# rdesc/autorally

Hardware: AMD Instinct MI355X
Metric: trajectory rollouts/s per MPPI solve (higher is better)
Workload: dtype f32

## Files before the change

autorally_amd/csrc/group_roles.hpp:

```cpp
#pragma once

#include "mppi_device.hpp"
#include "noise_device.hpp"

namespace mppi {

constexpr int kGRing = 16;
constexpr int kGCtlChunk = 4;

template <class SH>
struct GroupRoles {
  static constexpr int kPose = SH::NW, kCost = SH::NW + 1, kCtl = SH::NW + 2, kRng = SH::NW + 3;
  static constexpr int kWaves = SH::NW + 4;
  static_assert(kWaves <= (int)(sizeof(SH::fin) / sizeof(int)), "fin[]");
  static_assert(SH::kR == 16 || SH::kR == 8, "rollouts per group");
};
template <class SH>
__device__ __forceinline__ int group_j(int slot) { return slot & (SH::kR - 1); }
template <class SH>
__device__ __forceinline__ bool group_real(int slot) { return slot < SH::kR; }

template <class SH>
__device__ __forceinline__ int group_seq_min(SH &sh)
{
// ... 194 lines not shown
      y = fmaf(sd1, a.dt, y);
      yaw = fmaf(sd2, a.dt, yaw);
    }
    if (t > 0) {
      while (cdone < t - kGRing && --budget > 0) cdone = lds_peek(a_cd);
      if (lane < kRolloutsPerWave) *reinterpret_cast<float2 *>(&sh.tex[(t - 1) & (kGRing - 1)][lane][0]) = make_float2(tf_p, tb_p);
      lds_publish(a_mypub, t);
    }
    tf_p = tf; tb_p = tb;
  }
  spin_finish(budget, lds_addr(&sh.fail[0]), lds_addr(&sh.fin[R::kPose]));
}

template <int Q>
__device__ __forceinline__ float quad_bc(float v)
{
  return __int_as_float(__builtin_amdgcn_mov_dpp(__float_as_int(v), Q * 0x55, 0xF, 0xF, false));
}
__device__ __forceinline__ void quad_chain(float v, float d, float dt, int q, float &vq, float &v_out)
{
  const float v1 = fmaf(quad_bc<0>(d), dt, v);
  const float v2 = fmaf(quad_bc<1>(d), dt, v1);
  const float v3 = fmaf(quad_bc<2>(d), dt, v2);
  v_out = fmaf(quad_bc<3>(d), dt, v3);
  const float lo = (q == 0) ? v : v1, hi = (q == 2) ? v2 : v3;
  vq = (q < 2) ? lo : hi;
}
template <class SH, bool AFFINE>
__device__ __forceinline__ void group_pose_wave4(const RolloutArgs &a, SH &sh, const float x0, const float y0, const float yaw0,
                                                 const int budget_cut = 0);
template <class SH, bool AFFINE>
__device__ __forceinline__ void group_pose_wave4(const RolloutArgs &a, SH &sh)
{
  group_pose_wave4<SH, AFFINE>(a, sh, a.state[0], a.state[1], a.state[2]);
}
template <class SH, bool AFFINE>
__device__ __forceinline__ void group_pose_wave4(const RolloutArgs &a, SH &sh, const float x0, const float y0, const float yaw0,
                                                 const int budget_cut)
{
  using R = GroupRoles<SH>;
  constexpr int NSW = SH::NSW;
  static_assert(kRolloutsPerWave == 16 && kGRing >= 8, "lane = 4 j + q");
  const int lane = threadIdx.x & 63;
  const int j = group_j<SH>(lane >> 2), q = lane & 3;
  const int T = a.T;
  const uint32_t a_seq0 = lds_addr(&sh.xseq[0][0]);
  const uint32_t a_cd = lds_addr(&sh.cost_done[0]);
  const uint32_t a_mypub = lds_addr(&sh.pose_pub[lane]);
  float x = x0, y = y0, yaw = yaw0;
  int budget = spin_budget_init(a.spin_budget, T, a.fault_wave == R::kPose + 1 || budget_cut != 0), seen = 0, cdone = 0;
  for (int t0 = 0; t0 < T; t0 += 4) {
    const int t = t0 + q;
    const int tend = min(t0 + 4, T);
    const int need = (tend - 1) * NSW + 1;
    while (seen < need && --budget > 0) {
      seen = SH::kRecByAll ? group_seq_min(sh) : lds_peek(a_seq0);
      if (seen < need) __builtin_amdgcn_s_sleep(1);
    }
    const float4 r0 = *reinterpret_cast<const float4 *>(&sh.rec[t & (kGRing - 1)][j][0]);
    float yaw_q, yaw_n, x_q, x_n, y_q, y_n;
    quad_chain(yaw, a.negate_yaw_der ? -r0.w : r0.w, a.dt, q, yaw_q, yaw_n);
    float spsi, cpsi, tf = 0.0f, tb = 0.0f;
#ifdef MPPI_DIAG_NOPOSE
    spsi = 0.0f; cpsi = 1.0f;
#else
    sincos_fast(yaw_q, spsi, cpsi);
#endif
    quad_chain(x, fmaf(cpsi, r0.y, -(spsi * r0.z)), a.dt, q, x_q, x_n);
    quad_chain(y, fmaf(spsi, r0.y, cpsi * r0.z), a.dt, q, y_q, y_n);
#ifdef MPPI_DIAG_NOPOSE
    tf = x_q; tb = y_q;
#else
    const float st[3] = {x_q, y_q, yaw_q};
    track_fetch<AFFINE>(a.cost, st, cpsi, spsi, tf, tb);
#endif
    x = x_n; y = y_n; yaw = yaw_n;
    while (cdone < tend - kGRing && --budget > 0) cdone = lds_peek(a_cd);
    if (t < T) *reinterpret_cast<float2 *>(&sh.tex[t & (kGRing - 1)][j][0]) = make_float2(tf, tb);
    lds_publish(a_mypub, tend);
  }
  spin_finish(budget, lds_addr(&sh.fail[0]), lds_addr(&sh.fin[R::kPose]));
}

template <class SH>
__device__ __forceinline__ float group_settle(SH &sh, int budget, float J)
{
  using R = GroupRoles<SH>;
  const int lane = threadIdx.x & 63;
  const uint32_t a_fin = lds_addr(&sh.fin[(lane < R::kWaves) ? lane : 0]);
  for (;;) {
    const int v = (lane == R::kCost) ? 1 : lds_peek_lanes(a_fin);
    const bool all = __builtin_amdgcn_ballot_w64(v != 0) == ~0ull;
    if (all || --budget <= 0) break;
    __builtin_amdgcn_s_sleep(1);
  }
  if (budget <= 0 || lds_peek(lds_addr(&sh.fail[0])) != 0) J = __builtin_nanf("");
  return J;
}

template <class SH, bool CTRL>
__device__ __forceinline__ void group_cost_wave(const RolloutArgs &a, SH &sh)
{
  using R = GroupRoles<SH>;
  const int lane = threadIdx.x & 63;
  static_assert(SH::kR == 16, "one step per iteration: 16-rollout groups only");
  const int j = lane & 15;
  const int k = (int)blockIdx.x * kRolloutsPerWave + j;
// ... 2 lines not shown
  const uint32_t a_pose = lds_addr(&sh.pose_pub[0]);
  int crash = 0, budget = spin_budget_init(a.spin_budget, T, a.fault_wave == R::kCost + 1), seen = 0;
  float J = 0.0f;
  for (int t = 0; t < T; t++) {
    const double rt = a.inv_t[t];
    while (seen < t + 1 && --budget > 0) {
      seen = lds_peek(a_pose);
      if (seen < t + 1) __builtin_amdgcn_s_sleep(1);
    }
    const float4 r0 = *reinterpret_cast<const float4 *>(&sh.rec[t & (kGRing - 1)][j][0]);
    const float4 r1 = *reinterpret_cast<const float4 *>(&sh.ctl_rec[t & (kGRing - 1)][j][0]);
    const float2 tx = *reinterpret_cast<const float2 *>(&sh.tex[t & (kGRing - 1)][j][0]);
    lds_publish(a_mydone, t + 1);
    const int rc = (int)((t > 0) & (fabsf(r0.x) >= kRollCrash));
#ifdef MPPI_DIAG_NOCOST
    crash |= rc;
    int crash_new = crash;
    const float Jn = J + r0.y + r1.x + tx.x + (float)rt;
#else
    CostTerms ct;
    cost_terms_a<CTRL>(a.cost, a.nu, r0.y, r0.z, r1.x, r1.y, r1.z, r1.w, ct);
    crash |= rc;
    int crash_new = crash;
    const float c = cost_terms_b(a.cost, ct, tx.x, tx.y, crash_new);
    const float Jn = running_mean(J, c, t, rt);
#endif
    J = (t > 0) ? Jn : J;
    crash = (t > 0) ? crash_new : crash;
  }
  J = group_settle(sh, budget, J);
  a.costs[k] = J + 0.0f;
}

template <int Q>
__device__ __forceinline__ int quad_bc_i(int v)
{
  return __builtin_amdgcn_mov_dpp(v, Q * 0x55, 0xF, 0xF, false);
}
template <class SH, bool CTRL>
__device__ __forceinline__ void group_cost_wave4(const RolloutArgs &a, SH &sh)
{
  using R = GroupRoles<SH>;
  const int lane = threadIdx.x & 63;
  const int j = group_j<SH>(lane >> 2), q = lane & 3;
  const int k = (int)blockIdx.x * SH::kR + j;
  const int T = a.T;
  const uint32_t a_mydone = lds_addr(&sh.cost_done[lane]);
  const uint32_t a_pose = lds_addr(&sh.pose_pub[0]);
  int crash = 0, budget = spin_budget_init(a.spin_budget, T, a.fault_wave == R::kCost + 1), seen = 0;
  float J = 0.0f;
  for (int t0 = 0; t0 < T; t0 += 4) {
    const int t = t0 + q;
    const int tend = min(t0 + 4, T);
    while (seen < tend && --budget > 0) {
      seen = lds_peek(a_pose);
      if (seen < tend) __builtin_amdgcn_s_sleep(1);
    }
    const float4 r0 = *reinterpret_cast<const float4 *>(&sh.rec[t & (kGRing - 1)][j][0]);
    const float4 r1 = *reinterpret_cast<const float4 *>(&sh.ctl_rec[t & (kGRing - 1)][j][0]);
    const float2 tx = *reinterpret_cast<const float2 *>(&sh.tex[t & (kGRing - 1)][j][0]);
    lds_publish(a_mydone, tend);
    const bool counted = (t > 0) & (t < T);
    int e = (int)(fabsf(r0.x) >= kRollCrash) | (int)(tx.x >= a.cost.boundary_threshold) | (int)(tx.y >= a.cost.boundary_threshold);
    e = counted ? e : 0;
    const int c0 = crash | quad_bc_i<0>(e), c1 = c0 | quad_bc_i<1>(e), c2 = c1 | quad_bc_i<2>(e), c3 = c2 | quad_bc_i<3>(e);
    const int lo = (q == 0) ? c0 : c1, hi = (q == 2) ? c2 : c3;
    int crash_q = (q < 2) ? lo : hi;
    crash = c3;
#ifdef MPPI_DIAG_NOCOST
    const float c = r0.y + r1.x + tx.x + (float)crash_q;
#else
    CostTerms ct;
    cost_terms_a<CTRL>(a.cost, a.nu, r0.y, r0.z, r1.x, r1.y, r1.z, r1.w, ct);
    const float c = cost_terms_b(a.cost, ct, tx.x, tx.y, crash_q);
#endif
#pragma unroll
    for (int l = 0; l < 4; l++) {
      const int tl = t0 + l;
      const float cl = (l == 0) ? quad_bc<0>(c) : (l == 1) ? quad_bc<1>(c) : (l == 2) ? quad_bc<2>(c) : quad_bc<3>(c);
      if (tl > 0 && tl < T) {
#ifdef MPPI_DIAG_NOCOST
        J = J + cl + (float)a.inv_t[tl];
#else
        J = running_mean(J, cl, tl, a.inv_t[tl]);
#endif
      }
    }
  }
  J = group_settle(sh, budget, J);
  if (q == 0 && group_real<SH>(lane >> 2)) a.costs[k] = J + 0.0f;
}

}
```

autorally_amd/csrc/rollout_lds128.hip:

```cpp
#include "group_roles.hpp"
#include "m44_core.hpp"
#include "mppi_kernels.hpp"

namespace mppi {

struct Lds128Net {
  int n_layers;
  int layers[8];
};

struct Lds128Shared {
  static constexpr int NW = 4;
  static constexpr int NSW = 1;
  static constexpr int kR = 16;
  static constexpr bool kRecByAll = true;
  int xseq[NW][64];
  float rec[kGRing][kRolloutsPerWave][4];
  int cost_done[64];
  float ctl_b1[kGRing][64];
  float ctl_rec[kGRing][kRolloutsPerWave][4];
  int ctl_pub[64];
  float tex[kGRing][kRolloutsPerWave][2];
  int pose_pub[64];
  float eps[kGRing][kRolloutsPerWave][2];
  int rng_pub[64];
  int fail[4];
  int fin[8];
  float gstate[8];
  int gate_open[8];
  float dump[NW][64 * kGRing];
};
constexpr size_t kLds128ImageOffset = (sizeof(Lds128Shared) + 15) & ~(size_t)15;
constexpr size_t kLds128MaxBytes = 160 * 1024;

__host__ __device__ inline int lds128_quads_of(int nin) { return (nin + 3) >> 2; }
__host__ __device__ inline int lds128_halves_of(int nout) { return nout > 64 ? 2 : 1; }

__device__ __forceinline__ void lds128_pin_reads() { asm volatile("" ::: "memory"); }

template <int Q>
__device__ __forceinline__ void lds128_chain1(m44_f4 &d, const float (&T0)[4], const float (&T1)[4], m44_f4 (&w)[kLds44Ahead],
                                              const m44_f4 *p, const int nq)
{
  if constexpr (Q < 32) {
    if (Q > 0 && Q >= nq) return;
    const m44_f4 x = w[Q % kLds44Ahead];
    if constexpr (Q + kLds44Ahead < 32) w[Q % kLds44Ahead] = p[(Q + kLds44Ahead) * 64];
    lds128_pin_reads();
    const float (&T)[4] = Q < 16 ? T0 : T1;
    d = __builtin_amdgcn_mfma_f32_4x4x1f32(T[0], x[0], d, 4, Q & 15, 0);
    d = __builtin_amdgcn_mfma_f32_4x4x1f32(T[1], x[1], d, 4, Q & 15, 0);
    d = __builtin_amdgcn_mfma_f32_4x4x1f32(T[2], x[2], d, 4, Q & 15, 0);
    d = __builtin_amdgcn_mfma_f32_4x4x1f32(T[3], x[3], d, 4, Q & 15, 0);
    lds128_chain1<Q + 1>(d, T0, T1, w, p, nq);
  }
}

template <int Q>
__device__ __forceinline__ void lds128_chain2(m44_f4 &d0, m44_f4 &d1, const float (&T0)[4], const float (&T1)[4],
                                              m44_f4 (&w)[kLds44Ahead], const m44_f4 *p, const int nq)
{
  if constexpr (Q < 32) {
    if (Q > 0 && Q >= nq) return;
    constexpr int S = 2 * Q;
    const m44_f4 x0 = w[S % kLds44Ahead];
    if constexpr (S + kLds44Ahead < 64) w[S % kLds44Ahead] = p[(S + kLds44Ahead) * 64];
    const m44_f4 x1 = w[(S + 1) % kLds44Ahead];
    if constexpr (S + 1 + kLds44Ahead < 64) w[(S + 1) % kLds44Ahead] = p[(S + 1 + kLds44Ahead) * 64];
// ... 324 lines not shown
```

autorally_amd/csrc/rollout_lds44.hip:

```cpp
#include "group_roles.hpp"
#include "m44_core.hpp"
#include "mppi_kernels.hpp"

namespace mppi {

struct Lds44Net {
  int n_layers;
  int layers[8];
};

struct Lds44Shared {
  static constexpr int NW = 4;
  static constexpr int NSW = 1;
  static constexpr int kR = 16;
  static constexpr bool kRecByAll = true;
  int xseq[NW][64];
  float rec[kGRing][kRolloutsPerWave][4];
  int cost_done[64];
  float ctl_b1[kGRing][64];
  float ctl_rec[kGRing][kRolloutsPerWave][4];
  int ctl_pub[64];
  float tex[kGRing][kRolloutsPerWave][2];
  int pose_pub[64];
  float eps[kGRing][kRolloutsPerWave][2];
  int rng_pub[64];
  int fail[4];
  int fin[8];
  float gstate[8];
  int gate_open[8];
  float dump[NW][64 * kGRing];
};
constexpr size_t kLds44ImageOffset = (sizeof(Lds44Shared) + 15) & ~(size_t)15;

__host__ __device__ inline int lds44_quads_of(int nin) { return (nin + 3) >> 2; }

template <int Q>
__device__ __forceinline__ void lds44_chain(m44_f4 &d, const float (&T)[4], m44_f4 (&w)[kLds44Ahead], const m44_f4 *p, const int nq)
{
  if constexpr (Q < 16) {
    if (Q > 0 && Q >= nq) return;
    const m44_f4 x = w[Q % kLds44Ahead];
    if constexpr (Q + kLds44Ahead < 16) w[Q % kLds44Ahead] = p[(Q + kLds44Ahead) * 64];
    d = __builtin_amdgcn_mfma_f32_4x4x1f32(T[0], x[0], d, 4, Q, 0);
    d = __builtin_amdgcn_mfma_f32_4x4x1f32(T[1], x[1], d, 4, Q, 0);
    d = __builtin_amdgcn_mfma_f32_4x4x1f32(T[2], x[2], d, 4, Q, 0);
    d = __builtin_amdgcn_mfma_f32_4x4x1f32(T[3], x[3], d, 4, Q, 0);
    lds44_chain<Q + 1>(d, T, w, p, nq);
  }
}

template <bool GATED>
__device__ __forceinline__ void lds44_dynamics(const RolloutArgs &a, const Lds44Net &net, Lds44Shared &sh, const m44_f4 *img, const int w)
{
  const int lane = threadIdx.x & 63;
  const int i = lane & 3, row = lane >> 4;
  const int jr = 4 * w + i;
  const bool hi = (lane & 2) != 0, od = (lane & 1) != 0;
  const int T = a.T;
  const int n_w = net.n_layers - 1;
  const m44_f4 *pk = img + lane;
  const float *pb = reinterpret_cast<const float *>(pk);
  const m44_f4 w0a = pk[kLds44BiasQuads * 64], w0b = pk[(kLds44BiasQuads + 1) * 64];
  const float bs0 = pb[0];
  const float bo = pb[((n_w - 1) >> 2) * 256 + ((n_w - 1) & 3)];
  const m44_f4 *const p1 = pk + (kLds44BiasQuads + 2) * 64;
  unsigned long long nq_all = 0;
#pragma unroll
  for (int l = 1; l < 8; l++) nq_all |= (unsigned long long)lds44_quads_of(net.layers[l]) << (5 * l);
// ... 250 lines not shown
```

autorally_amd/csrc/rollout_m44.hip:

```cpp
#include "group_roles.hpp"
#include "m44_core.hpp"
#include "mppi_kernels.hpp"

namespace mppi {

constexpr int kM44H = 64;

struct M44Shared {
  static constexpr int NW = 4;
  static constexpr int NSW = 1;
  static constexpr int kR = 16;
  static constexpr bool kRecByAll = true;
  int xseq[NW][64];
  float rec[kGRing][kRolloutsPerWave][4];
  int cost_done[64];
  float ctl_b1[kGRing][64];
  float ctl_rec[kGRing][kRolloutsPerWave][4];
  int ctl_pub[64];
  float tex[kGRing][kRolloutsPerWave][2];
  int pose_pub[64];
  float eps[kGRing][kRolloutsPerWave][2];
  int rng_pub[64];
  int fail[4];
  int fin[8];
  float gstate[8];
  int gate_open[8];
  m44_f4 wo[4][64];
  float dump[NW][64 * kGRing];
};

template <int NHID>
constexpr int m44_q_bias() { return 2; }
template <int NHID>
constexpr int m44_q_hidden() { return 2 + (NHID + 3) / 4; }
template <int NHID>
constexpr int m44_q_out() { return m44_q_hidden<NHID>() + (NHID - 1) * 16; }
template <int NHID>
constexpr int m44_q_total() { return m44_q_out<NHID>() + 5; }

template <int K>
__device__ __forceinline__ void m44_step(m44_f4 &d, const float (&T)[4], const float *w)
{
  d = __builtin_amdgcn_mfma_f32_4x4x1f32(T[K & 3], w[K], d, 4, K >> 2, 0);
}
template <int K0>
__device__ __forceinline__ void m44_steps16(m44_f4 &d, const float (&T)[4], const float *w)
{
#define S4(K) m44_step<K>(d, T, w); m44_step<K + 1>(d, T, w); m44_step<K + 2>(d, T, w); m44_step<K + 3>(d, T, w);
  S4(K0) S4(K0 + 4) S4(K0 + 8) S4(K0 + 12)
#undef S4
}
template <int CTRL>
__device__ __forceinline__ float m44_dpp_add(float acc, float src)
{
  return acc + __int_as_float(__builtin_amdgcn_update_dpp(0, __float_as_int(src), CTRL, 0xF, 0xF, true));
}
__device__ __forceinline__ float m44_out_tree(const f32x2 (&q)[4], const f32x2 (&p)[4], const float (&T)[4])
{
  f32x2 Q = q[0] * f32x2{T[0], T[0]}, P = p[0] * f32x2{T[0], T[0]};
#pragma unroll
  for (int s = 1; s < 4; s++) {
    Q = __builtin_elementwise_fma(q[s], f32x2{T[s], T[s]}, Q);
    P = __builtin_elementwise_fma(p[s], f32x2{T[s], T[s]}, P);
  }
  {
// ... 300 lines not shown
```

autorally_amd/csrc/rollout_oct.hip:

```cpp
#include "mfma_net.hpp"
#include "group_roles.hpp"
#include "mppi_kernels.hpp"

namespace mppi {

template <int H, int NHID>
struct OctShared {
  static constexpr int NW = 4;
  static constexpr int NSW = NHID;
  static constexpr int kR = 16;
  static constexpr bool kRecByAll = false;
  float xb[2][NW][64][4];
  int xseq[NW][64];
  float rec[kGRing][kRolloutsPerWave][4];
  int cost_done[64];
  float ctl_b1[kGRing][64];
  float ctl_rec[kGRing][kRolloutsPerWave][4];
  int ctl_pub[64];
  float tex[kGRing][kRolloutsPerWave][2];
  int pose_pub[64];
  float eps[kGRing][kRolloutsPerWave][2];
  int rng_pub[64];
  int fail[4];
  int fin[8];
};

__device__ __forceinline__ void oct_poll(const uint32_t (&a_seq)[3], const uint32_t (&a_x)[3], int &f, f32x4 (&oth)[3])
{
  int f0, f1, f2;
  asm volatile(
      "ds_read_b32 %0, %6\n\tds_read_b128 %3, %9\n\t"
      "ds_read_b32 %1, %7\n\tds_read_b128 %4, %10\n\t"
      "ds_read_b32 %2, %8\n\tds_read_b128 %5, %11\n\t"
      "s_waitcnt lgkmcnt(0)"
      : "=&v"(f0), "=&v"(f1), "=&v"(f2), "=&v"(oth[0]), "=&v"(oth[1]), "=&v"(oth[2])
      : "v"(a_seq[0]), "v"(a_seq[1]), "v"(a_seq[2]), "v"(a_x[0]), "v"(a_x[1]), "v"(a_x[2])
      : "memory");
  f = __builtin_amdgcn_readfirstlane(min(min(f0, f1), f2));
}

template <int H, int NHID, int W>
__device__ __forceinline__ void oct_dynamics(const RolloutArgs &a, OctShared<H, NHID> &sh)
{
  using N = MfmaNet<H, NHID>;
  constexpr int MT = N::MT, KSH = N::KSH, NSW = NHID;
  static_assert(MT == 4, "one M tile per dynamics wave: 64-wide hidden layers");
  const int lane = threadIdx.x & 63;
  const int j = lane & 15, g = lane >> 4;
  const int T = a.T;

  float A0[2], B0[4], AH[(NHID - 1) * KSH + 1], Bh[(NHID - 1) * 4 + 1], AL[KSH], BL[4];
  A0[0] = a.wpack[(W * 2 + 0) * 64 + lane];
  A0[1] = a.wpack[(W * 2 + 1) * 64 + lane];
#pragma unroll
  for (int r = 0; r < 4; r++) B0[r] = a.wpack[(N::nA + W * 4 + r) * 64 + lane] * kTanhScale;
#pragma unroll
  for (int l = 1; l < NHID; l++) {
#pragma unroll
    for (int s = 0; s < KSH; s++)
      AH[(l - 1) * KSH + s] = a.wpack[(N::nA0 + (l - 1) * N::nAH + W * KSH + s) * 64 + lane];
#pragma unroll
    for (int r = 0; r < 4; r++) Bh[(l - 1) * 4 + r] = a.wpack[(N::nA + l * MT * 4 + W * 4 + r) * 64 + lane] * kTanhScale;
  }
#pragma unroll
// ... 170 lines not shown
```

autorally_amd/csrc/rollout_row.hip:

```cpp
#include "group_roles.hpp"
#include "mppi_kernels.hpp"

namespace mppi {

#ifdef MPPI_ROW_STAMPS
__device__ unsigned long long g_row_stamps[16];
#define RSTAMP(i)                                                                                         \
  do {                                                                                                    \
    if (blockIdx.x == 0 && (threadIdx.x & 63) == 0) {                                                     \
      unsigned long long t__;                                                                             \
      asm volatile("s_memtime %0\n\ts_waitcnt lgkmcnt(0)" : "=s"(t__)::"memory");                           \
      g_row_stamps[i] = t__;                                                                              \
    }                                                                                                     \
  } while (0)
#else
#define RSTAMP(i) do { } while (0)
#endif

template <int H>
struct RowShared {
  static constexpr int NW = 4;
  static constexpr int NSW = 1;
  static constexpr bool kRecByAll = true;
  static constexpr int kR = 16;
  int xseq[NW][64];
  float rec[kGRing][kRolloutsPerWave][4];
  int cost_done[64];
  float ctl_b1[kGRing][64];
  float ctl_rec[kGRing][kRolloutsPerWave][4];
  int ctl_pub[64];
  float tex[kGRing][kRolloutsPerWave][2];
  int pose_pub[64];
  float eps[kGRing][kRolloutsPerWave][2];
  int rng_pub[64];
  int fail[4];
  int fin[8];
  float gstate[8];
  int gate_open[8];
  float dump[NW][64 * 2 + (kGRing - 1) * kRolloutsPerWave * 4];
};

template <int H, bool TREE>
struct RowWeights {
  f32x2 w1[kNetIn], w2[H], w3[TREE ? 4 : H];
  f32x2 b1s, b2s, b3;
};

constexpr int kRowPackEntries = 40;
template <int H, bool TREE>
__device__ __forceinline__ void row_load(const float *rowpack, int p, RowWeights<H, TREE> &W)
{
  static_assert(H == 32, "entry layout of pack_row_weights");
  const float4 *pk = reinterpret_cast<const float4 *>(rowpack) + p;
#pragma unroll
  for (int i = 0; i < 3; i++) {
    const float4 v = pk[i * 16];
    W.w1[2 * i] = f32x2{v.x, v.y};
    W.w1[2 * i + 1] = f32x2{v.z, v.w};
  }
#pragma unroll
  for (int i = 0; i < H / 2; i++) {
    const float4 v = pk[(3 + i) * 16];
    W.w2[2 * i] = f32x2{v.x, v.y};
    W.w2[2 * i + 1] = f32x2{v.z, v.w};
    if constexpr (!TREE) {
      const float4 u = pk[(3 + H / 2 + i) * 16];
      W.w3[2 * i] = f32x2{u.x, u.y};
      W.w3[2 * i + 1] = f32x2{u.z, u.w};
    }
  }
  const float4 b = pk[35 * 16];
  W.b1s = f32x2{b.x, b.y};
  W.b2s = f32x2{b.z, b.w};
  if constexpr (TREE) {
    const float4 u = pk[37 * 16], v = pk[38 * 16], c = pk[39 * 16];
    W.w3[0] = f32x2{u.x, u.y};
// ... 7 lines not shown
  }
}

template <int Q>
__device__ __forceinline__ float row_bc(float a)
{
  return __int_as_float(__builtin_amdgcn_mov_dpp(__float_as_int(a), 0x150 + Q, 0xF, 0xF, false));
}
template <int Q>
__device__ __forceinline__ f32x2 row_bc2(f32x2 a)
{
  return __builtin_bit_cast(f32x2, (long long)__builtin_amdgcn_mov_dpp(__builtin_bit_cast(long long, a), 0x150 + Q, 0xF, 0xF, false));
}
template <int Q>
__device__ __forceinline__ void row_dot_step(f32x2 &z, f32x2 &b, const f32x2 *w, f32x2 a)
{
  z = __builtin_elementwise_fma(w[2 * Q], f32x2{b.x, b.x}, z);
  __builtin_amdgcn_sched_barrier(0);
  const f32x2 bn = row_bc2<(Q + 1 < 16 ? Q + 1 : 15)>(a);
  __builtin_amdgcn_sched_barrier(0);
  z = __builtin_elementwise_fma(w[2 * Q + 1], f32x2{b.y, b.y}, z);
  __builtin_amdgcn_sched_barrier(0);
  b = bn;
}
__device__ __forceinline__ f32x2 row_dot_bc(const f32x2 *w, f32x2 a)
{
  f32x2 z = {0.0f, 0.0f};
  f32x2 b = row_bc2<0>(a);
  __builtin_amdgcn_sched_barrier(0);
#define RD4(Q) row_dot_step<Q>(z, b, w, a); row_dot_step<Q + 1>(z, b, w, a); row_dot_step<Q + 2>(z, b, w, a); row_dot_step<Q + 3>(z, b, w, a);
  RD4(0) RD4(4) RD4(8) RD4(12)
#undef RD4
  return z;
}

template <int CTRL>
__device__ __forceinline__ float dpp_add(float acc, float src)
{
  return acc + __int_as_float(__builtin_amdgcn_update_dpp(0, __float_as_int(src), CTRL, 0xF, 0xF, true));
}
__device__ __forceinline__ float row_out_tree(const f32x2 *w3, f32x2 a)
{
  const f32x2 ax = {a.x, a.x}, ay = {a.y, a.y};
  const f32x2 v01 = __builtin_elementwise_fma(w3[1], ay, w3[0] * ax);
  const f32x2 v23 = __builtin_elementwise_fma(w3[3], ay, w3[2] * ax);
  float v0 = dpp_add<0x128>(v01.x, v23.x);
  const float v1 = dpp_add<0x128>(v01.y, v23.y);
  v0 = dpp_add<0x141>(v0, v1);
  v0 = dpp_add<0xB1>(v0, v0);
  v0 = dpp_add<0x4E>(v0, v0);
  return v0;
}

template <int H, bool TREE, int Q>
__device__ __forceinline__ void row_step(const RolloutArgs &a, const RowWeights<H, TREE> &W, f32x2 &sp, f32x2 &un, const int t0,
                                         const uint32_t a_rec, const uint32_t a_myseq, const volatile int __attribute__((address_space(3))) *p_pub,
                                         const volatile f32x2 __attribute__((address_space(3))) *&pu,
                                         const volatile f32x2 __attribute__((address_space(3))) *p_u0, int &cp, int &budget)
{
  constexpr int kSlotF2 = kRolloutsPerWave * 2;
  constexpr uint32_t kRecStride = sizeof(float) * kRolloutsPerWave * 4;
  const int t = t0 + Q;
  const f32x2 u = un;
  const f32x2 slo = TREE ? f32x2{row_bc<0>(sp.x), row_bc<4>(sp.x)} : f32x2{row_bc<0>(sp.x), row_bc<0>(sp.y)};
  const f32x2 shi = TREE ? f32x2{row_bc<8>(sp.x), row_bc<12>(sp.x)} : f32x2{row_bc<1>(sp.x), row_bc<1>(sp.y)};
  if constexpr (TREE) asm volatile("ds_write_b32 %0, %1 offset:%2" ::"v"(a_rec), "v"(sp.x), "n"(Q * kRecStride) : "memory");
  else asm volatile("ds_write_b64 %0, %1 offset:%2" ::"v"(a_rec), "v"(sp), "n"(Q * kRecStride) : "memory");
  if constexpr (Q == 3) lds_publish(a_myseq, t + 1);
  f32x2 z = {0.0f, 0.0f};
  z = __builtin_elementwise_fma(W.w1[0], f32x2{slo.x, slo.x}, z);
  z = __builtin_elementwise_fma(W.w1[1], f32x2{slo.y, slo.y}, z);
  z = __builtin_elementwise_fma(W.w1[2], f32x2{shi.x, shi.x}, z);
  z = __builtin_elementwise_fma(W.w1[3], f32x2{shi.y, shi.y}, z);
  z = __builtin_elementwise_fma(W.w1[4], f32x2{u.x, u.x}, z);
  z = __builtin_elementwise_fma(W.w1[5], f32x2{u.y, u.y}, z);
  int cp_v = 0;
  if constexpr (Q == 0) cp_v = *p_pub;
  if constexpr (Q == 3) pu = p_u0 + ((t + 1) & (kGRing - 1)) * kSlotF2;
  constexpr int kUn = (Q == 3) ? 0 : (Q + 1) * kSlotF2;
  un = pu[kUn];
  const f32x2 a0 = tanh_bias2(z, W.b1s);
  const f32x2 a1 = tanh_bias2(row_dot_bc(W.w2, a0), W.b2s);
  const int want = t + 2;
  if constexpr (Q == 0) cp = __builtin_amdgcn_readfirstlane(cp_v);
  asm volatile("" : "+v"(un));
  if constexpr (TREE) {
    const float d = row_out_tree(W.w3, a1) + W.b3.x;
    sp.x = fmaf(d, a.dt, sp.x);
    asm volatile("" : "+v"(sp.x));
  } else {
    const f32x2 d = row_dot_bc(W.w3, a1) + W.b3;
    sp = __builtin_elementwise_fma(d, f32x2{a.dt, a.dt}, sp);
    asm volatile("" : "+v"(sp));
  }
  if (__builtin_expect(cp < want, 0)) {
    while (cp < want && --budget > 0) {
      cp = __builtin_amdgcn_readfirstlane(*p_pub);
      un = pu[kUn];
    }
    asm volatile("" : "+v"(un));
  }
}

template <int H, bool TREE, bool GATED = false>
__device__ __forceinline__ void row_dynamics(const RolloutArgs &a, RowShared<H> &sh, const int w)
{
  static_assert(H == 32, "row_dot_bc: 32 activations, two per lane of a 16-lane row");
  static_assert(kGRing % 4 == 0, "aligned chunks of four steps inside the ring");
  const int lane = threadIdx.x & 63;
  const int r = lane >> 4, p = lane & 15;
  const int jr = 4 * w + r;
  const bool odd = (p & 1) != 0;
  const int T = a.T;
  RowWeights<H, TREE> W;
  row_load<H, TREE>(a.wpack, p, W);
#pragma unroll
  for (int k = 0; k < H; k++) asm volatile("" : "+v"(W.w2[k]));
#pragma unroll
  for (int k = 0; k < (TREE ? 4 : H); k++) asm volatile("" : "+v"(W.w3[k]));

  const uint32_t a_myseq = lds_addr(&sh.xseq[w][lane]);
  typedef const volatile int __attribute__((address_space(3))) *lds_int_p;
  typedef const volatile f32x2 __attribute__((address_space(3))) *lds_f2_p;
  const lds_int_p p_pub = (lds_int_p)&sh.ctl_pub[0];
  uint32_t a_u0 = lds_addr(&sh.ctl_rec[0][jr][0]);
  asm volatile("" : "+v"(a_u0));
  const lds_f2_p p_u = (lds_f2_p)a_u0;
  const uint32_t a_rec0 = TREE ? (((p & 3) == 0) ? lds_addr(&sh.rec[0][jr][p >> 2]) : lds_addr(&sh.dump[w][2 * lane]))
                               : ((p < 2) ? lds_addr(&sh.rec[0][jr][2 * p]) : lds_addr(&sh.dump[w][2 * lane]));
  constexpr uint32_t kRecStride = sizeof(float) * kRolloutsPerWave * 4;

  int budget = spin_budget_init(a.spin_budget, T, a.fault_wave == w + 1);
  f32x2 sp;
  if constexpr (GATED) {
    const uint32_t a_go = lds_addr(&sh.gate_open[0]);
    while (lds_peek(a_go) == 0 && --budget > 0) __builtin_amdgcn_s_sleep(1);
    const volatile float *gs = sh.gstate;
    sp = TREE ? f32x2{gs[3 + (p >> 2)], 0.0f} : odd ? f32x2{gs[5], gs[6]} : f32x2{gs[3], gs[4]};
  } else {
    sp = TREE ? f32x2{a.state[3 + (p >> 2)], 0.0f} : odd ? f32x2{a.state[5], a.state[6]} : f32x2{a.state[3], a.state[4]};
  }
  if (w == 0) RSTAMP(2);
  int cp = 0;
  while ((cp = __builtin_amdgcn_readfirstlane(*p_pub)) < 1 && --budget > 0) __builtin_amdgcn_s_sleep(1);
  if (w == 0) RSTAMP(3);
  lds_f2_p pu = p_u;
  f32x2 un = pu[0];
  asm volatile("" : "+v"(un));

  const int NS = T - 1;
  for (int t0 = 0; t0 < NS; t0 += 4) {
    const uint32_t a_rec = a_rec0 + (uint32_t)(t0 & (kGRing - 1)) * kRecStride;
    row_step<H, TREE, 0>(a, W, sp, un, t0, a_rec, a_myseq, p_pub, pu, p_u, cp, budget);
    if (t0 + 1 >= NS) break;
    row_step<H, TREE, 1>(a, W, sp, un, t0, a_rec, a_myseq, p_pub, pu, p_u, cp, budget);
    if (t0 + 2 >= NS) break;
    row_step<H, TREE, 2>(a, W, sp, un, t0, a_rec, a_myseq, p_pub, pu, p_u, cp, budget);
    if (t0 + 3 >= NS) break;
    row_step<H, TREE, 3>(a, W, sp, un, t0, a_rec, a_myseq, p_pub, pu, p_u, cp, budget);
  }
  if (w == 0) RSTAMP(4);
  {
    const int t = T - 1;
    if constexpr (TREE) asm volatile("ds_write_b32 %0, %1" ::"v"(a_rec0 + (uint32_t)(t & (kGRing - 1)) * kRecStride), "v"(sp.x) : "memory");
    else asm volatile("ds_write_b64 %0, %1" ::"v"(a_rec0 + (uint32_t)(t & (kGRing - 1)) * kRecStride), "v"(sp) : "memory");
    lds_publish(a_myseq, t + 1);
  }
  spin_finish(budget, lds_addr(&sh.fail[0]), lds_addr(&sh.fin[w]));
}

template <int H, bool AFFINE, bool CTRL, bool TREE, bool GATED = false>
__device__ __forceinline__ void row_group(const RolloutArgs &a, RowShared<H> &sh)
{
  using SH = RowShared<H>;
  using R = GroupRoles<SH>;
  const int lane = threadIdx.x & 63;
  const int role = __builtin_amdgcn_readfirstlane(threadIdx.x >> 6);
  if (role == 0) RSTAMP(0);
  MrgHalf g0{0, 0, 0};
  if (role == R::kRng) g0 = group_rng_load<SH>(a);
  if (role == 0) {
#pragma unroll
    for (int w = 0; w < 4; w++) sh.xseq[w][lane] = 0;
    sh.cost_done[lane] = 0;
    sh.ctl_pub[lane] = 0;
    sh.pose_pub[lane] = 0;
    sh.rng_pub[lane] = 0;
    sh.fail[lane & 3] = 0;
    sh.fin[lane & 7] = 0;
    sh.gate_open[lane & 7] = 0;
  }
  __syncthreads();
  if (role == 0) RSTAMP(1);
#ifdef MPPI_ROW_RIDER_PRIO
  if (role >= 4) __builtin_amdgcn_s_setprio(MPPI_ROW_RIDER_PRIO);
#endif
  if (role < 4) row_dynamics<H, TREE, GATED>(a, sh, role);
  else if (role == R::kCost) { group_cost_wave4<SH, CTRL>(a, sh); RSTAMP(5); }
  else if (role == R::kCtl) { group_control_wave(a, sh, GATED ? lds_addr(&sh.gate_open[0]) : 0u); RSTAMP(6); }
  else if (role == R::kPose) {
    if constexpr (GATED) {
      const int shut = group_gate_wait(a, sh);
      const volatile float *gs = sh.gstate;
      const float x0 = gs[0], y0 = gs[1], yaw0 = gs[2];
      group_pose_wave4<SH, AFFINE>(a, sh, x0, y0, yaw0, shut);
    } else {
      group_pose_wave4<SH, AFFINE>(a, sh);
    }
    RSTAMP(7);
  }
  else { group_rng_wave<SH, true>(a, sh, g0); RSTAMP(8); }
}
// ... 118 lines not shown
```

autorally_amd/csrc/rollout_row64.hip:

```cpp
#include "group_roles.hpp"
#include "mppi_kernels.hpp"

namespace mppi {

constexpr int kH64 = 64;
constexpr int kPF = 8;

template <int NHID, int R>
struct Row64Shared {
  static constexpr int NW = R / 2;
  static constexpr int NSW = 1;
  static constexpr int kR = R;
  static constexpr bool kRecByAll = true;
  f32x2 wl[NHID - 1][kH64][32];
  int xseq[NW][64];
  float rec[kGRing][kRolloutsPerWave][4];
  int cost_done[64];
  float ctl_b1[kGRing][64];
  float ctl_rec[kGRing][kRolloutsPerWave][4];
  int ctl_pub[64];
  float tex[kGRing][kRolloutsPerWave][2];
  int pose_pub[64];
  float eps[kGRing][kRolloutsPerWave][2];
  int rng_pub[64];
  int fail[4];
  int fin[16];
  float dump[NW][64 * kGRing];
};

template <int NHID>
struct Row64Regs {
  f32x2 w1[kNetIn];
  f32x2 bs[NHID];
  f32x2 q[2], p[2];
  float bo;
};
template <int NHID>
constexpr int row64_reg_entries() { return 3 + (NHID + 1) / 2 + 3; }

template <int NHID>
__device__ __forceinline__ void row64_load(const float *pack, int g, Row64Regs<NHID> &W)
{
  constexpr int NB = (NHID + 1) / 2;
  const float4 *pk = reinterpret_cast<const float4 *>(pack) + g;
#pragma unroll
  for (int i = 0; i < 3; i++) {
    const float4 v = pk[i * 32];
    W.w1[2 * i] = f32x2{v.x, v.y};
    W.w1[2 * i + 1] = f32x2{v.z, v.w};
  }
#pragma unroll
  for (int i = 0; i < NB; i++) {
    const float4 v = pk[(3 + i) * 32];
    W.bs[2 * i] = f32x2{v.x, v.y};
    if (2 * i + 1 < NHID) W.bs[2 * i + 1] = f32x2{v.z, v.w};
  }
  const float4 u = pk[(3 + NB) * 32], v = pk[(4 + NB) * 32], c = pk[(5 + NB) * 32];
  W.q[0] = f32x2{u.x, u.y};
  W.q[1] = f32x2{u.z, u.w};
  W.p[0] = f32x2{v.x, v.y};
  W.p[1] = f32x2{v.z, v.w};
  W.bo = c.x;
}

template <int Q>
__device__ __forceinline__ float r64_bc(float a)
// ... 237 lines not shown
```

autorally_amd/csrc/solve_kernels.hip:

```cpp
#include "mppi_device.hpp"
#include "mppi_kernels.hpp"


namespace mppi {


#ifdef MPPI_TAIL_STAMPS
__device__ unsigned long long g_tail_stamps[16];
#define TSTAMP(i)                                                                                   \
  do {                                                                                              \
    if (block == T / 2 && threadIdx.x == 0) {                                                       \
      unsigned long long t__;                                                                       \
      asm volatile("s_memrealtime %0\n\ts_waitcnt lgkmcnt(0)" : "=s"(t__)::"memory");               \
      g_tail_stamps[i] = t__;                                                                       \
    }                                                                                               \
  } while (0)
#else
#define TSTAMP(i) do { } while (0)
#endif
#ifndef MPPI_TAIL_THREADS
#define MPPI_TAIL_THREADS 512
#endif
constexpr int kTailThreads = MPPI_TAIL_THREADS;
constexpr int kRedChunk = 4096;
// ... 98 lines not shown
    for (int i = tid; i < T * 2; i += kTailThreads) {
      float acc = f0 * X[i];
      float p = f1 * X[i + 2];
      acc = acc + p;
      p = f2 * X[i + 4];
      acc = acc + p;
      p = f1 * X[i + 6];
      acc = acc + p;
      p = f0 * X[i + 8];
      acc = acc + p;
      a.U[i] = acc;
      Y[i] = acc;
    }
    if (a.hist_out != nullptr && tid < 4) a.hist_out[tid] = X[tid];
  }
  __syncthreads();

  if (a.slid != nullptr) {
    const int st = a.slide_stride;
    const float init_j = (tid & 1) ? a.init1 : a.init0;
    for (int i = tid; i < 2 * T; i += kTailThreads) {
      const int r = i >> 1, j = i & 1;
      a.slid[i] = (r < T - st) ? Y[(r + st) * 2 + j] : init_j;
    }
    if (tid < 4) {
      float hv;
      if (st == 1) hv = (tid < 2) ? X[tid + 2] : Y[tid - 2];
      else hv = Y[(st - 2) + tid];
      a.slid[2 * T + tid] = hv;
    }
  }
}

__device__ __forceinline__ void solve_tail_body(const TailArgs &a, const int block, const float *V, const float *costs_p, const int K,
                                                const int T)
{
  constexpr int kGS = 68, kPlane = (kRedChunk / 64) * kGS;
  __shared__ __attribute__((aligned(16))) float tile[2][kPlane];
  __shared__ __attribute__((aligned(16))) float wtile[kPlane];
  __shared__ float redm[kTailThreads / 64], reds[kTailThreads / 64], redt[kTailThreads / 64];
  __shared__ int is_last;
  extern __shared__ __attribute__((aligned(16))) float dyn[];
  float *partial = dyn;
  const int tid = threadIdx.x;
  const bool extra = (block == T);
  const int t = extra ? 0 : block;
  constexpr int base = 0;
  const int n = K;
  TSTAMP(0);

  const float *row = V + ((size_t)t * K + base) * 2;
  constexpr int kPre = kRedChunk / 2 / kTailThreads;
  float4 pre[kPre];
  {
    const float4 *src0 = reinterpret_cast<const float4 *>(row);
#pragma unroll
    for (int i = 0; i < kPre; i++) {
      const int q = tid + i * kTailThreads;
      pre[i] = (q < n / 2) ? src0[q] : make_float4(0, 0, 0, 0);
    }
  }
  float eta;
  {
    constexpr int kCostV = kRedChunk / 4 / kTailThreads;
    const float4 *c4 = reinterpret_cast<const float4 *>(costs_p);
    const int K4 = K / 4;
    float4 cv[kCostV];
#pragma unroll
    for (int i = 0; i < kCostV; i++) {
      const int q = i * kTailThreads + tid;
      cv[i] = (q < K4) ? c4[q] : make_float4(INFINITY, INFINITY, INFINITY, INFINITY);
    }
    float m = INFINITY;
    TSTAMP(1);
#pragma unroll
    for (int i = 0; i < kCostV; i++) m = fminf(fminf(m, fminf(cv[i].x, cv[i].y)), fminf(cv[i].z, cv[i].w));
    TSTAMP(2);
    const float beta = block_reduce<true>(m, redm);
    TSTAMP(3);
    float part = 0.0f;
#pragma unroll
    for (int i = 0; i < kCostV; i++) {
      const int q = i * kTailThreads + tid;
      if (q < K4) {
        const float e0 = expf(-a.gamma * (cv[i].x - beta));
        const float e1 = expf(-a.gamma * (cv[i].y - beta));
        const float e2 = expf(-a.gamma * (cv[i].z - beta));
        const float e3 = expf(-a.gamma * (cv[i].w - beta));
        cv[i] = make_float4(e0, e1, e2, e3);
        part += (e0 + e1) + (e2 + e3);
      }
    }
    TSTAMP(4);
    eta = block_reduce<false>(part, reds);
    TSTAMP(5);
    if (extra) {
      float tc = 0.0f;
#pragma unroll
      for (int i = 0; i < kCostV; i++) {
        const int q = i * kTailThreads + tid;
        if (q < K4) {
          reinterpret_cast<float4 *>(a.w)[q] = cv[i];
          tc += cv[i].x * cv[i].x / eta;
          tc += cv[i].y * cv[i].y / eta;
          tc += cv[i].z * cv[i].z / eta;
          tc += cv[i].w * cv[i].w / eta;
        }
      }
      const float traj = block_reduce<false>(tc, redt);
      if (tid == 0) {
        __hip_atomic_store(&a.scal[0], beta, __ATOMIC_RELAXED, __HIP_MEMORY_SCOPE_AGENT);
        __hip_atomic_store(&a.scal[1], eta, __ATOMIC_RELAXED, __HIP_MEMORY_SCOPE_AGENT);
        __hip_atomic_store(&a.scal[2], traj, __ATOMIC_RELAXED, __HIP_MEMORY_SCOPE_AGENT);
        if (a.last_iter) {
          publish_entry(a.res, T, beta, eta, a.seq);
          publish_entry(a.res, T + 1, traj, 0.0f, a.seq);
        }
      }
    } else {
#pragma unroll
      for (int i = 0; i < kCostV; i++) {
        const int q = i * kTailThreads + tid;
        const int kl = 4 * q - base;
        if (q < K4 && kl >= 0 && kl < n)
          *reinterpret_cast<float4 *>(&wtile[(kl >> 6) * kGS + (kl & 63)]) =
              make_float4(cv[i].x / eta, cv[i].y / eta, cv[i].z / eta, cv[i].w / eta);
      }
    }
  }

  const int G = K / 64;
  if (!extra) {
#pragma unroll
    for (int i = 0; i < kPre; i++) {
      const int q = tid + i * kTailThreads;
      if (q < n / 2) {
        const int kk = 2 * q;
        const int o = (kk >> 6) * kGS + (kk & 63);
        *reinterpret_cast<float2 *>(&tile[0][o]) = make_float2(pre[i].x, pre[i].z);
        *reinterpret_cast<float2 *>(&tile[1][o]) = make_float2(pre[i].y, pre[i].w);
      }
    }
    TSTAMP(6);
    __syncthreads();
    TSTAMP(7);
    for (int c = tid; c < (n / 64) * 2; c += kTailThreads) {
      const int ml = c >> 1, j = c & 1;
      const float4 *p4 = reinterpret_cast<const float4 *>(&tile[j][ml * kGS]);
      const float4 *w4 = reinterpret_cast<const float4 *>(&wtile[ml * kGS]);
      float acc = 0.0f;
#pragma unroll
      for (int i = 0; i < 16; i++) {
        const float4 wv = w4[i], pv = p4[i];
        acc = fmaf(wv.x, pv.x, acc);
        acc = fmaf(wv.y, pv.y, acc);
        acc = fmaf(wv.z, pv.z, acc);
        acc = fmaf(wv.w, pv.w, acc);
      }
      partial[j * G + ml] = acc;
    }
    TSTAMP(8);
    __syncthreads();
  }
  float u = 0.0f;
  if (tid < 2 && !extra) {
    const float *pj = partial + tid * G;
    int mm = 0;
    if ((G & 3) == 0) {
      for (; mm + 32 <= G; mm += 32) {
        float4 v[8];
#pragma unroll
        for (int i = 0; i < 8; i++) v[i] = *reinterpret_cast<const float4 *>(pj + mm + 4 * i);
#pragma unroll
        for (int i = 0; i < 8; i++) { u += v[i].x; u += v[i].y; u += v[i].z; u += v[i].w; }
      }
    }
    for (; mm < G; mm++) u += pj[mm];
    if (a.last_iter) store_granule(a.ug + t * 2 + tid, a.seq, u);
    else a.U[t * 2 + tid] = u;
  }
  if (tid < 64) {
    const float u1 = __shfl(u, 1);
    TSTAMP(9);
    if (tid == 0 && !extra && a.last_iter) publish_entry(a.res, t, u, u1, a.seq);
    TSTAMP(10);
  }
  tail_arrive_and_smooth(a, K, T, (unsigned)(T + 1), is_last, dyn);
}

#ifdef MPPI_TAIL_STAMPS
__device__ unsigned long long g_stream_stamps[2][16];
#define SSTAMP(i)                                                                                   \
  do {                                                                                              \
    if (t == T / 2 && (closer || c == 0) && threadIdx.x == 0) {                                     \
      unsigned long long t__;                                                                       \
      asm volatile("s_memrealtime %0\n\ts_waitcnt lgkmcnt(0)" : "=s"(t__)::"memory");               \
      g_stream_stamps[closer ? 0 : 1][i] = t__;                                                     \
    }                                                                                               \
  } while (0)
#else
#define SSTAMP(i) do { } while (0)
#endif
#ifndef MPPI_STREAM_SLEEP
#define MPPI_STREAM_SLEEP 1
#endif
constexpr int kMaxChunks = 64;
constexpr int kBcastReplicas = 32;
constexpr int kGxSumReplicas = 3 * kMaxChunks + kBcastReplicas * 16;
static_assert(kTailExchangeGranules == kGxSumReplicas + kBcastReplicas * kMaxChunks, "mppi_kernels.hpp");
static_assert(2 * kBcastReplicas <= kTailThreads, "one lane per replica granule");
struct StreamTailArgs {
  TailArgs a;
  unsigned long long *gx;
  unsigned long long *gpart;
  unsigned epoch;
  unsigned poll_ticks;
  int fault;
};


__device__ __forceinline__ void poll_replica(const unsigned long long *g, const unsigned epoch, const unsigned long long t0,
                                             const unsigned poll_ticks, float *out)
{
  if (threadIdx.x < 64) {
    float v = 0.0f;
    bool ok = threadIdx.x != 0;
    for (;;) {
      if (!ok) {
        const unsigned long long x = __hip_atomic_load(g, __ATOMIC_RELAXED, __HIP_MEMORY_SCOPE_AGENT);
        if ((unsigned)(x >> 32) == epoch) { v = __uint_as_float((unsigned)x); ok = true; }
      }
      if (__all(ok)) break;
// ... 536 lines not shown
```

Measured before the change: 106.8 million.

## Shorten last-step dependency chain in row rollout and move tail tile writes earlier

In the row rollout kernel the final dynamics step is peeled off: it publishes its sequence immediately and skips the next-control load. The pose and cost waves gain an early-last path in which pose waits only for step T-2, and cost polls every dynamics wave's sequence word through a ballot instead of waiting on pose. The solve tail kernel now issues the V row loads together with the cost loads, writes the LDS tile before the eta reduction rather than after it, and clamps out-of-range indices instead of branching. It also skips the granule store when no_device_copy is set. These changes aim to shorten serialized waits at the end of the horizon and overlap memory loads with the reduction, at the cost of more complex synchronization whose correctness at the last step is harder to check.

```diff
diff --git a/autorally_amd/csrc/group_roles.hpp b/autorally_amd/csrc/group_roles.hpp
--- a/autorally_amd/csrc/group_roles.hpp
+++ b/autorally_amd/csrc/group_roles.hpp
@@ -270,7 +270,8 @@
   for (int t0 = 0; t0 < T; t0 += 4) {
     const int t = t0 + q;
     const int tend = min(t0 + 4, T);
-    const int need = (tend - 1) * NSW + 1;
+    int need = (tend - 1) * NSW + 1;
+    if (SH::kEarlyLast && tend == T && T >= 2) need = (T - 2) * NSW + 1;
     while (seen < need && --budget > 0) {
       seen = SH::kRecByAll ? group_seq_min(sh) : lds_peek(a_seq0);
       if (seen < need) __builtin_amdgcn_s_sleep(1);
@@ -379,9 +380,20 @@
   for (int t0 = 0; t0 < T; t0 += 4) {
     const int t = t0 + q;
     const int tend = min(t0 + 4, T);
-    while (seen < tend && --budget > 0) {
-      seen = lds_peek(a_pose);
-      if (seen < tend) __builtin_amdgcn_s_sleep(1);
+    if (SH::kEarlyLast && tend == T) {
+      static_assert(!SH::kEarlyLast || SH::kRecByAll, "every dynamics wave writes records: all NW words are looked at");
+      const uint32_t a_look = (lane < SH::NW) ? lds_addr(&sh.xseq[lane < SH::NW ? lane : 0][0]) : a_pose;
+      const int want = (lane < SH::NW) ? (T - 1) * SH::NSW + 1 : tend;
+      bool there = false;
+      while (!there && --budget > 0) {
+        there = __builtin_amdgcn_ballot_w64(lds_peek_lanes(a_look) >= want) == ~0ull;
+        if (!there) __builtin_amdgcn_s_sleep(1);
+      }
+    } else {
+      while (seen < tend && --budget > 0) {
+        seen = lds_peek(a_pose);
+        if (seen < tend) __builtin_amdgcn_s_sleep(1);
+      }
     }
     const float4 r0 = *reinterpret_cast<const float4 *>(&sh.rec[t & (kGRing - 1)][j][0]);
     const float4 r1 = *reinterpret_cast<const float4 *>(&sh.ctl_rec[t & (kGRing - 1)][j][0]);
diff --git a/autorally_amd/csrc/rollout_lds128.hip b/autorally_amd/csrc/rollout_lds128.hip
--- a/autorally_amd/csrc/rollout_lds128.hip
+++ b/autorally_amd/csrc/rollout_lds128.hip
@@ -14,6 +14,7 @@
   static constexpr int NSW = 1;
   static constexpr int kR = 16;
   static constexpr bool kRecByAll = true;
+  static constexpr bool kEarlyLast = false;
   int xseq[NW][64];
   float rec[kGRing][kRolloutsPerWave][4];
   int cost_done[64];
diff --git a/autorally_amd/csrc/rollout_lds44.hip b/autorally_amd/csrc/rollout_lds44.hip
--- a/autorally_amd/csrc/rollout_lds44.hip
+++ b/autorally_amd/csrc/rollout_lds44.hip
@@ -14,6 +14,7 @@
   static constexpr int NSW = 1;
   static constexpr int kR = 16;
   static constexpr bool kRecByAll = true;
+  static constexpr bool kEarlyLast = false;
   int xseq[NW][64];
   float rec[kGRing][kRolloutsPerWave][4];
   int cost_done[64];
diff --git a/autorally_amd/csrc/rollout_m44.hip b/autorally_amd/csrc/rollout_m44.hip
--- a/autorally_amd/csrc/rollout_m44.hip
+++ b/autorally_amd/csrc/rollout_m44.hip
@@ -11,6 +11,7 @@
   static constexpr int NSW = 1;
   static constexpr int kR = 16;
   static constexpr bool kRecByAll = true;
+  static constexpr bool kEarlyLast = false;
   int xseq[NW][64];
   float rec[kGRing][kRolloutsPerWave][4];
   int cost_done[64];
diff --git a/autorally_amd/csrc/rollout_oct.hip b/autorally_amd/csrc/rollout_oct.hip
--- a/autorally_amd/csrc/rollout_oct.hip
+++ b/autorally_amd/csrc/rollout_oct.hip
@@ -10,6 +10,7 @@
   static constexpr int NSW = NHID;
   static constexpr int kR = 16;
   static constexpr bool kRecByAll = false;
+  static constexpr bool kEarlyLast = false;
   float xb[2][NW][64][4];
   int xseq[NW][64];
   float rec[kGRing][kRolloutsPerWave][4];
diff --git a/autorally_amd/csrc/rollout_row.hip b/autorally_amd/csrc/rollout_row.hip
--- a/autorally_amd/csrc/rollout_row.hip
+++ b/autorally_amd/csrc/rollout_row.hip
@@ -22,6 +22,7 @@
   static constexpr int NW = 4;
   static constexpr int NSW = 1;
   static constexpr bool kRecByAll = true;
+  static constexpr bool kEarlyLast = true;
   static constexpr int kR = 16;
   int xseq[NW][64];
   float rec[kGRing][kRolloutsPerWave][4];
@@ -135,7 +136,7 @@
   return v0;
 }
 
-template <int H, bool TREE, int Q>
+template <int H, bool TREE, int Q, bool LAST = false>
 __device__ __forceinline__ void row_step(const RolloutArgs &a, const RowWeights<H, TREE> &W, f32x2 &sp, f32x2 &un, const int t0,
                                          const uint32_t a_rec, const uint32_t a_myseq, const volatile int __attribute__((address_space(3))) *p_pub,
                                          const volatile f32x2 __attribute__((address_space(3))) *&pu,
@@ -149,7 +150,8 @@
   const f32x2 shi = TREE ? f32x2{row_bc<8>(sp.x), row_bc<12>(sp.x)} : f32x2{row_bc<1>(sp.x), row_bc<1>(sp.y)};
   if constexpr (TREE) asm volatile("ds_write_b32 %0, %1 offset:%2" ::"v"(a_rec), "v"(sp.x), "n"(Q * kRecStride) : "memory");
   else asm volatile("ds_write_b64 %0, %1 offset:%2" ::"v"(a_rec), "v"(sp), "n"(Q * kRecStride) : "memory");
-  if constexpr (Q == 3) lds_publish(a_myseq, t + 1);
+  if constexpr (Q == 3 && !LAST) lds_publish(a_myseq, t + 1);
+  if constexpr (LAST) lds_publish(a_myseq, t + 1);
   f32x2 z = {0.0f, 0.0f};
   z = __builtin_elementwise_fma(W.w1[0], f32x2{slo.x, slo.x}, z);
   z = __builtin_elementwise_fma(W.w1[1], f32x2{slo.y, slo.y}, z);
@@ -161,7 +163,7 @@
   if constexpr (Q == 0) cp_v = *p_pub;
   if constexpr (Q == 3) pu = p_u0 + ((t + 1) & (kGRing - 1)) * kSlotF2;
   constexpr int kUn = (Q == 3) ? 0 : (Q + 1) * kSlotF2;
-  un = pu[kUn];
+  if constexpr (!LAST) un = pu[kUn];
   const f32x2 a0 = tanh_bias2(z, W.b1s);
   const f32x2 a1 = tanh_bias2(row_dot_bc(W.w2, a0), W.b2s);
   const int want = t + 2;
@@ -179,7 +181,7 @@
   if (__builtin_expect(cp < want, 0)) {
     while (cp < want && --budget > 0) {
       cp = __builtin_amdgcn_readfirstlane(*p_pub);
-      un = pu[kUn];
+      if constexpr (!LAST) un = pu[kUn];
     }
     asm volatile("" : "+v"(un));
   }
@@ -232,15 +234,19 @@
   asm volatile("" : "+v"(un));
 
   const int NS = T - 1;
-  for (int t0 = 0; t0 < NS; t0 += 4) {
+  for (int t0 = 0; t0 < NS - 1; t0 += 4) {
     const uint32_t a_rec = a_rec0 + (uint32_t)(t0 & (kGRing - 1)) * kRecStride;
     row_step<H, TREE, 0>(a, W, sp, un, t0, a_rec, a_myseq, p_pub, pu, p_u, cp, budget);
-    if (t0 + 1 >= NS) break;
+    if (t0 + 1 >= NS - 1) break;
     row_step<H, TREE, 1>(a, W, sp, un, t0, a_rec, a_myseq, p_pub, pu, p_u, cp, budget);
-    if (t0 + 2 >= NS) break;
+    if (t0 + 2 >= NS - 1) break;
     row_step<H, TREE, 2>(a, W, sp, un, t0, a_rec, a_myseq, p_pub, pu, p_u, cp, budget);
-    if (t0 + 3 >= NS) break;
+    if (t0 + 3 >= NS - 1) break;
     row_step<H, TREE, 3>(a, W, sp, un, t0, a_rec, a_myseq, p_pub, pu, p_u, cp, budget);
+  }
+  if (NS >= 1) {
+    const int t = NS - 1;
+    row_step<H, TREE, 0, true>(a, W, sp, un, t, a_rec0 + (uint32_t)(t & (kGRing - 1)) * kRecStride, a_myseq, p_pub, pu, p_u, cp, budget);
   }
   if (w == 0) RSTAMP(4);
   {
diff --git a/autorally_amd/csrc/rollout_row64.hip b/autorally_amd/csrc/rollout_row64.hip
--- a/autorally_amd/csrc/rollout_row64.hip
+++ b/autorally_amd/csrc/rollout_row64.hip
@@ -12,6 +12,7 @@
   static constexpr int NSW = 1;
   static constexpr int kR = R;
   static constexpr bool kRecByAll = true;
+  static constexpr bool kEarlyLast = false;
   f32x2 wl[NHID - 1][kH64][32];
   int xseq[NW][64];
   float rec[kGRing][kRolloutsPerWave][4];
diff --git a/autorally_amd/csrc/solve_kernels.hip b/autorally_amd/csrc/solve_kernels.hip
--- a/autorally_amd/csrc/solve_kernels.hip
+++ b/autorally_amd/csrc/solve_kernels.hip
@@ -174,14 +174,6 @@
   const float *row = V + ((size_t)t * K + base) * 2;
   constexpr int kPre = kRedChunk / 2 / kTailThreads;
   float4 pre[kPre];
-  {
-    const float4 *src0 = reinterpret_cast<const float4 *>(row);
-#pragma unroll
-    for (int i = 0; i < kPre; i++) {
-      const int q = tid + i * kTailThreads;
-      pre[i] = (q < n / 2) ? src0[q] : make_float4(0, 0, 0, 0);
-    }
-  }
   float eta;
   {
     constexpr int kCostV = kRedChunk / 4 / kTailThreads;
@@ -192,6 +184,14 @@
     for (int i = 0; i < kCostV; i++) {
       const int q = i * kTailThreads + tid;
       cv[i] = (q < K4) ? c4[q] : make_float4(INFINITY, INFINITY, INFINITY, INFINITY);
+    }
+    {
+      const float4 *src0 = reinterpret_cast<const float4 *>(row);
+#pragma unroll
+      for (int i = 0; i < kPre; i++) {
+        const int q = tid + i * kTailThreads;
+        pre[i] = src0[(q < n / 2) ? q : 0];
+      }
     }
     float m = INFINITY;
     TSTAMP(1);
@@ -214,6 +214,19 @@
       }
     }
     TSTAMP(4);
+    if (!extra) {
+#pragma unroll
+      for (int i = 0; i < kPre; i++) {
+        const int q = tid + i * kTailThreads;
+        if (q < n / 2) {
+          const int kk = 2 * q;
+          const int o = (kk >> 6) * kGS + (kk & 63);
+          *reinterpret_cast<float2 *>(&tile[0][o]) = make_float2(pre[i].x, pre[i].z);
+          *reinterpret_cast<float2 *>(&tile[1][o]) = make_float2(pre[i].y, pre[i].w);
+        }
+      }
+    }
+    TSTAMP(6);
     eta = block_reduce<false>(part, reds);
     TSTAMP(5);
     if (extra) {
@@ -253,17 +266,6 @@
 
   const int G = K / 64;
   if (!extra) {
-#pragma unroll
-    for (int i = 0; i < kPre; i++) {
-      const int q = tid + i * kTailThreads;
-      if (q < n / 2) {
-        const int kk = 2 * q;
-        const int o = (kk >> 6) * kGS + (kk & 63);
-        *reinterpret_cast<float2 *>(&tile[0][o]) = make_float2(pre[i].x, pre[i].z);
-        *reinterpret_cast<float2 *>(&tile[1][o]) = make_float2(pre[i].y, pre[i].w);
-      }
-    }
-    TSTAMP(6);
     __syncthreads();
     TSTAMP(7);
     for (int c = tid; c < (n / 64) * 2; c += kTailThreads) {
@@ -298,8 +300,8 @@
       }
     }
     for (; mm < G; mm++) u += pj[mm];
-    if (a.last_iter) store_granule(a.ug + t * 2 + tid, a.seq, u);
-    else a.U[t * 2 + tid] = u;
+    if (!a.last_iter) a.U[t * 2 + tid] = u;
+    else if (!a.no_device_copy) store_granule(a.ug + t * 2 + tid, a.seq, u);
   }
   if (tid < 64) {
     const float u1 = __shfl(u, 1);
```

Measured after the change: 108.7 million, median of 6. 1.02x the previous value.
